# meuleman/epilogos

Hardware: AMD Instinct MI355X
Metric: Mbins scored/sec (S1, 18-state, 833 biosamples) (higher is better)
Workload: dtype u8

## Files before the change

epilogos_amd/csrc/epg_common.h:

```cpp
#pragma once
#include <hip/hip_runtime.h>
#include <stdarg.h>
#include <stdint.h>
#include <stdio.h>

#include <type_traits>

#include "epilogos_amd.h"

typedef unsigned int u32;
typedef unsigned long long u64;
typedef unsigned short u16;

namespace epg {

int fail(int code, const char* fmt, ...);
int num_cus();

#ifdef EPILOGOS_BUILD_EXPERIMENTS
#include <stdlib.h>
static inline const char* exp_env(const char* name) { return getenv(name); }
#else
static inline const char* exp_env(const char*) { return nullptr; }
#endif

enum Force { FORCE_NULL_SEQ = 0, FORCE_S3_SCORE_BINS, FORCE_S3_CONTRACTION, FORCE_S3_HIST_LDS, FORCE_K1_BLOCKS_PER_CU, FORCE_CUS, FORCE_COUNT };
extern int g_force[FORCE_COUNT];

#define EPG_HIP(expr)                                                                         \
    do {                                                                                      \
        hipError_t _e = (expr);                                                               \
        if (_e != hipSuccess)                                                                 \
            return epg::fail(EPG_ERR_HIP, "%s failed: %s", #expr, hipGetErrorString(_e));     \
    } while (0)

#define EPG_LAUNCH_CHECK(name)                                                                \
    do {                                                                                      \
        hipError_t _e = hipGetLastError();                                                    \
        if (_e != hipSuccess)                                                                 \
            return epg::fail(EPG_ERR_HIP, "launch of %s failed: %s", name, hipGetErrorString(_e)); \
    } while (0)

static inline int64_t align_up(int64_t x, int64_t a) { return (x + a - 1) / a * a; }

template <int DEFAULT, typename F>
static inline auto with_constant(int, F&& f) {
    return f(std::integral_constant<int, DEFAULT>{});
}
template <int DEFAULT, int V, int... VS, typename F>
static inline auto with_constant(int v, F&& f) {
    if (v == V) return f(std::integral_constant<int, V>{});
    return with_constant<DEFAULT, VS...>(v, f);
}

int64_t s1_ws_bytes(int64_t R, int N, int S);
int grid_for_tiles(long R);
long fast_rows(long R, int N, long ldx);
int64_t s2_table_bytes(int maxc, int S);
int64_t s3_ws_bytes(int64_t R, int N, int S);
int64_t s3_xt_bytes(int64_t R, int N);
int transpose_states(const char* X, int64_t R, int32_t N, int64_t ldx, int32_t S, char* XT, int64_t Rp, int shift, int bad, int* dirty,
                     hipStream_t st);
int64_t s3_gemm_ws_bytes(int64_t R, int N, int S);
int64_t s3_gemm_ws_min_bytes(int64_t R, int N, int S);
int hist_s3_gemm(const char* X, int64_t R, int32_t N, int64_t ldx, int32_t S, int32_t* counts, void* ws, int64_t ws_bytes, hipStream_t st);
bool s3_lanes_ok(int N, int S);
int64_t s3_lanes_ws_bytes(int64_t R, int N, int S);
int score_s3_lanes(const int8_t* X8, int64_t R, int32_t N, int64_t ldx, int32_t S, const float* q, double* out64, float* out32, void* ws,
                   int64_t ws_bytes, hipStream_t st);
int wide_hist_s2_from_binhist(const uint16_t* H, const uint16_t* H2, int64_t R, int32_t S, int64_t* counts, hipStream_t st);
int wide_score_s2_from_hist(const uint16_t* H, int64_t R, int32_t S, int64_t perms, const float* q, double* out64, float* out32, hipStream_t st);
int wide_hist_s3(const int8_t* X, int64_t R, int32_t N, int64_t ldx, int32_t S, int32_t* counts, hipStream_t st);
int wide_score_s3(const int8_t* X, int64_t R, int32_t N, int64_t ldx, int32_t S, const float* q, double* out64, float* out32, void* ws,
                  int64_t ws_bytes, hipStream_t st);

struct DynLds {
    unsigned long long done = 0;
};
static inline hipError_t ensure_dyn_lds(DynLds& a, const void* kernel, int bytes) {
    int dev = 0;
    hipError_t e = hipGetDevice(&dev);
    if (e != hipSuccess) return e;
    const unsigned long long bit = 1ull << (dev & 63);
    if (__atomic_load_n(&a.done, __ATOMIC_ACQUIRE) & bit) return hipSuccess;
    e = hipFuncSetAttribute(kernel, hipFuncAttributeMaxDynamicSharedMemorySize, bytes);
    if (e == hipSuccess) __atomic_fetch_or(&a.done, bit, __ATOMIC_RELEASE);
    return e;
}

static inline int tile_rows(int64_t row_bytes) {
    int tr = 64;
    while (tr > 8 && 4 * tr * row_bytes > 65536) tr >>= 1;
    return tr;
}

__device__ __forceinline__ u32 bfi(u32 m, u32 a, u32 b) { return (a & m) | (b & ~m); }

__device__ __forceinline__ uint4 ld16(const char* p) {
    uint4 v;
    __builtin_memcpy(&v, p, 16);
    return v;
}

__device__ __forceinline__ u32 quad_sum(u32 v) {
    v += (u32)__builtin_amdgcn_update_dpp(0, (int)v, 0xB1, 0xf, 0xf, false);
    v += (u32)__builtin_amdgcn_update_dpp(0, (int)v, 0x4E, 0xf, 0xf, false);
    return v;
}

__device__ __forceinline__ void store_staged(const char* lds, char* dst, int nbytes, int lane) {
    const int nchunks = nbytes >> 4;
    for (int c = lane; c < nchunks; c += 64)
        *reinterpret_cast<uint4*>(dst + 16 * c) = *reinterpret_cast<const uint4*>(lds + 16 * c);
    const int tail0 = nchunks << 4;
    for (int o = tail0 + 4 * lane; o + 4 <= nbytes; o += 256)
        *reinterpret_cast<u32*>(dst + o) = *reinterpret_cast<const u32*>(lds + o);
    if ((nbytes & 2) && lane == 0) *reinterpret_cast<u16*>(dst + nbytes - 2) = *reinterpret_cast<const u16*>(lds + nbytes - 2);
}

typedef u32 epg_u32x4 __attribute__((ext_vector_type(4)));
__device__ __forceinline__ void store_staged_nt(const char* lds, char* dst, int nbytes, int lane) {
    const int nchunks = nbytes >> 4;
    for (int c = lane; c < nchunks; c += 64)
        __builtin_nontemporal_store(*reinterpret_cast<const epg_u32x4*>(lds + 16 * c), reinterpret_cast<epg_u32x4*>(dst + 16 * c));
    const int tail0 = nchunks << 4;
    for (int o = tail0 + 4 * lane; o + 4 <= nbytes; o += 256)
        __builtin_nontemporal_store(*reinterpret_cast<const u32*>(lds + o), reinterpret_cast<u32*>(dst + o));
    if ((nbytes & 2) && lane == 0) *reinterpret_cast<u16*>(dst + nbytes - 2) = *reinterpret_cast<const u16*>(lds + nbytes - 2);
}

__device__ __forceinline__ double kl_term(double p, double q) {
    if (q == 0.0) return 0.0;
    const double r = p / q;
    if (!(r > 0.0)) return 0.0;
    return p * log2(r);
}

__device__ __forceinline__ float s3_table_entry(float qv, float obs) {
    if (qv == 0.0f) return 0.0f;
    const float r = __fdiv_rn(obs, qv);
    if (!(r > 0.0f)) return 0.0f;
#ifdef EPG_S3_TABLE_LOG2F
    return obs * log2f(r);
#else
    return __fmul_rn(obs, (float)log2((double)r));
#endif
}

}
```

epilogos_amd/csrc/epg_s1.hip:

```cpp
#include "epg_count.h"
#include "epg_paircount.h"

#include <stdlib.h>
#include <string.h>

namespace epg {

constexpr int K1P_LD = 17;

template <int SC, bool FULL, bool PAIRS, typename Loop>
__device__ __forceinline__ void bin_hist_body(int Sout_, u64* __restrict__ counts, int nmax, u64* __restrict__ counts2, Loop&& loop) {
    constexpr int S = SC;
    constexpr int ND = (S + 1) / 2;
    const int Sout = FULL ? S : Sout_;
    const int ROWB = 2 * Sout;
    __shared__ u64 s_cnt[S + 1];
    __shared__ __attribute__((aligned(16))) char s_stage[4][32 * 2 * S];
    constexpr int PG = (S + 2) / 3, PSP = 3 * PG, PROLES = PG * (PG + 1) / 2, PSLICE = PROLES <= 64 ? 64 / PROLES : 1;
    static_assert(!PAIRS || (FULL && PROLES <= 64), "the pair counts need a compile-time row width and at most 64 block roles");
    __shared__ u32 s_pair[PAIRS ? 4 * PSP * K1P_LD : 1];
    __shared__ u64 s_c2[PAIRS ? S * S : 1];
    const int lane = threadIdx.x & 63, wave = threadIdx.x >> 6;
    const int j = lane & 3, b = lane >> 2;
    if (threadIdx.x <= S) s_cnt[threadIdx.x] = 0;
    if (PAIRS) {
        for (int e = threadIdx.x; e < S * S; e += 256) s_c2[e] = 0;
        for (int e = threadIdx.x; e < 4 * PSP * K1P_LD; e += 256) s_pair[e] = 0;
    }
    __syncthreads();
    u16* H = nullptr;
    int pgi = -1, pgj = 0, pkq = 0;
    u64 pacc[PAIRS ? 9 : 1], prs[PAIRS ? 3 : 1];
    if (PAIRS) {
        const int role = lane < PROLES * PSLICE ? lane / PSLICE : -1;
        pkq = lane % PSLICE;
        if (role >= 0) pair_role(role, PG, pgi, pgj);
#pragma unroll
        for (int c = 0; c < 9; ++c) pacc[c] = 0;
#pragma unroll
        for (int c = 0; c < 3; ++c) prs[c] = 0;
    }
    auto pair_counts = [&](const char* stage, int rows) {
        u32* sp = s_pair + wave * PSP * K1P_LD;
        const u16* raw = reinterpret_cast<const u16*>(stage);
        __builtin_amdgcn_wave_barrier();
        for (int e = lane; e < S * 16; e += 64) {
            const int i = e >> 4, k = e & 15;
            const u32 lo = 2 * k < rows ? raw[(2 * k) * S + i] : 0u, hi = 2 * k + 1 < rows ? raw[(2 * k + 1) * S + i] : 0u;
            sp[i * K1P_LD + k] = lo | (hi << 16);
        }
        __builtin_amdgcn_wave_barrier();
        if (pgi >= 0) {
            u32 part[9], ps[3];
            pair_tile_dot(sp + 3 * pgi * K1P_LD, sp + 3 * pgj * K1P_LD, K1P_LD, pkq, 16, PSLICE, pgi == pgj, part, ps);
#pragma unroll
            for (int c = 0; c < 9; ++c) pacc[c] += part[c];
#pragma unroll
            for (int c = 0; c < 3; ++c) prs[c] += ps[c];
        }
        __builtin_amdgcn_wave_barrier();
    };

    StateTotals<S> totals;
    totals.init(nmax);

    auto enter = [&](u16* Hpart) { H = Hpart; };
    auto epilogue = [&](int half, long row, bool valid, u32 (&cnt)[S]) {
        u32 d[ND];
        pack_reduce<S>(cnt, d);
        if (counts) totals.add(d, valid, s_cnt, j);
        if (H) stage_hist_row<S, FULL && (S & 1) == 0>(&s_stage[wave][(half * 16 + b) * ROWB], d, j, Sout);
    };
    auto finish = [&](long st, long row0, int rows) {
        if (H) store_staged(s_stage[wave], reinterpret_cast<char*>(H) + row0 * ROWB, rows * ROWB, lane);
        if constexpr (PAIRS) pair_counts(s_stage[wave], rows);
    };
    loop(enter, epilogue, finish);

    if (counts) totals.commit(s_cnt, j, counts, Sout);
    if constexpr (PAIRS) {
        if (pgi >= 0) pair_fold(pacc, prs, pgi, pgj, S, s_c2);
        pair_commit(s_c2, S, counts2);
    }
}

template <int SC, int NG, bool FULL>
__global__ __launch_bounds__(256) void k_bin_hist(const char* __restrict__ X, long R, int N, long ldx, int Sout_,
                                                   u16* __restrict__ H, u64* __restrict__ counts) {
    bin_hist_body<SC, FULL, false>(Sout_, counts, N, nullptr, [&](auto&& enter, auto&& epilogue, auto&& finish) {
        enter(H);
        tile_loop<SC, NG>(X, R, N, ldx, epilogue, finish);
    });
}

template <int SC, int NG>
__global__ __launch_bounds__(256) void k_bin_hist_s2(const char* __restrict__ X, long R, int N, long ldx, u16* __restrict__ H,
                                                      u64* __restrict__ counts, u64* __restrict__ counts2) {
    bin_hist_body<SC, true, true>(SC, counts, N, counts2, [&](auto&& enter, auto&& epilogue, auto&& finish) {
        enter(H);
        tile_loop<SC, NG>(X, R, N, ldx, epilogue, finish);
    });
}

template <int SC, int NG, bool FULL>
__global__ __launch_bounds__(256) void k_bin_hist_parts(const KhParts pt, int Sout_, u64* __restrict__ counts, int nmax) {
    bin_hist_body<SC, FULL, false>(Sout_, counts, nmax, nullptr, [&](auto&& enter, auto&& epilogue, auto&& finish) {
        tile_loop_parts<SC, NG>(pt, [&](int part) { enter(pt.h[part]); }, epilogue, finish);
    });
}

__global__ __launch_bounds__(256) void k_bin_hist_safe(const char* __restrict__ X, long row_begin, long row_end, int N,
                                                        long ldx, int S, u16* __restrict__ H, u64* __restrict__ counts, int mask = 31) {
    __shared__ u32 s_h[4][128];
    const int lane = threadIdx.x & 63, wave = threadIdx.x >> 6;
    for (long row = row_begin + (long)blockIdx.x * 4 + wave; row < row_end; row += (long)gridDim.x * 4) {
        for (int s = lane; s < S; s += 64) s_h[wave][s] = 0;
        __builtin_amdgcn_wave_barrier();
        const char* rp = X + row * ldx;
        for (int n = lane; n < N; n += 64) {
            const int v = (unsigned char)rp[n] & mask;
            if (v < S) atomicAdd(&s_h[wave][v], 1u);
        }
        __builtin_amdgcn_wave_barrier();
        for (int s = lane; s < S; s += 64) {
            const u32 c = s_h[wave][s];
            if (H) H[row * S + s] = (u16)c;
            if (counts && c) atomicAdd(&counts[s], (u64)c);
        }
        __builtin_amdgcn_wave_barrier();
    }
}

__global__ void k_s1_table(const float* __restrict__ q, int N, int S, double* __restrict__ T64, float* __restrict__ T32) {
    const long e = (long)blockIdx.x * blockDim.x + threadIdx.x;
    if (e >= (long)(N + 1) * S) return;
    const int c = (int)(e / S), s = (int)(e % S);
    const double p = (double)c / (double)N;
    const double v = kl_term(p, (double)q[s]);
    T64[e] = v;
    T32[e] = (float)v;
}

template <int S, int NG, typename OT>
__global__ __launch_bounds__(256) void k_score_s1(const char* __restrict__ X, long R, int N, long ldx,
                                                   const OT* __restrict__ T, OT* __restrict__ out) {
    constexpr int ND = (S + 1) / 2;
    constexpr int ROWB = S * (int)sizeof(OT);
    __shared__ __attribute__((aligned(16))) char s_stage[4][32 * ROWB];
    const int lane = threadIdx.x & 63, wave = threadIdx.x >> 6;
    const int j = lane & 3, b = lane >> 2;
    auto epilogue = [&](int half, long row, bool valid, u32 (&cnt)[S]) {
        u32 d[ND];
        pack_reduce<S>(cnt, d);
        OT* srow = reinterpret_cast<OT*>(&s_stage[wave][(half * 16 + b) * ROWB]);
#pragma unroll
        for (int k = 0; k < (S + 3) / 4; ++k) {
            const u32 c = quad_state_count(d, k, j);
            const int s = 4 * k + j;
            if (s < S) srow[s] = (c && valid) ? T[(long)c * S + s] : (OT)0;
        }
    };
    auto finish = [&](long st, long row0, int rows) {
        store_staged_nt(s_stage[wave], reinterpret_cast<char*>(out) + row0 * ROWB, rows * ROWB, lane);
    };
    tile_loop<S, NG>(X, R, N, ldx, epilogue, finish);
}

template <typename OT, bool LDS_T>
__global__ __launch_bounds__(LDS_T ? 1024 : 256) void k_score_s1_from_hist(const u16* __restrict__ H, long total, int S,
                                                                             const OT* __restrict__ Tg, int nent, OT* __restrict__ out,
                                                                             u64* __restrict__ zero_counts, int rev) {
    extern __shared__ __attribute__((aligned(16))) char smem_t[];
    if (zero_counts && blockIdx.x == 0 && (int)threadIdx.x < S) zero_counts[threadIdx.x] = 0;
    const OT* T = Tg;
    if (LDS_T) {
        OT* Ts = reinterpret_cast<OT*>(smem_t);
        for (int e = threadIdx.x; e < nent; e += blockDim.x) Ts[e] = Tg[e];
        __syncthreads();
        T = Ts;
    }
    const u32 cmax = (u32)(nent / S - 1);
    const long nquads = total >> 2;
    const long stride = (long)gridDim.x * blockDim.x;
    long qd = (long)blockIdx.x * blockDim.x + threadIdx.x;
    const long qtop = nquads - 1, qsgn = rev ? -1 : 1, qoff = rev ? qtop : 0;
    for (; qd + 3 * stride < nquads; qd += 4 * stride) {
        uint2 h[4];
#pragma unroll
        for (int u = 0; u < 4; ++u) h[u] = *reinterpret_cast<const uint2*>(H + 4 * (qoff + qsgn * (qd + u * stride)));
#pragma unroll
        for (int u = 0; u < 4; ++u) {
            const long e0 = 4 * (qoff + qsgn * (qd + u * stride));
            int s = (int)(e0 % S);
            const u32 c[4] = {h[u].x & 0xffffu, h[u].x >> 16, h[u].y & 0xffffu, h[u].y >> 16};
            OT v[4];
#pragma unroll
            for (int k = 0; k < 4; ++k) {
                v[k] = c[k] - 1u < cmax ? T[(long)c[k] * S + s] : (OT)0;
                s = s + 1 == S ? 0 : s + 1;
            }
            if constexpr (sizeof(OT) == 4) {
                typedef float v4f_nt __attribute__((ext_vector_type(4)));
                const v4f_nt vv = {(float)v[0], (float)v[1], (float)v[2], (float)v[3]};
                __builtin_nontemporal_store(vv, reinterpret_cast<v4f_nt*>(out + e0));
            } else {
                typedef double v2d_nt __attribute__((ext_vector_type(2)));
                const v2d_nt lo = {(double)v[0], (double)v[1]}, hi = {(double)v[2], (double)v[3]};
                __builtin_nontemporal_store(lo, reinterpret_cast<v2d_nt*>(out + e0));
                __builtin_nontemporal_store(hi, reinterpret_cast<v2d_nt*>(out + e0 + 2));
            }
        }
    }
    for (; qd < nquads; qd += stride) {
        const long e0 = 4 * (qoff + qsgn * qd);
        int s = (int)(e0 % S);
        for (int k = 0; k < 4; ++k) {
            const u32 c = H[e0 + k];
            out[e0 + k] = c - 1u < cmax ? T[(long)c * S + s] : (OT)0;
            s = s + 1 == S ? 0 : s + 1;
        }
    }
    if (blockIdx.x == 0 && threadIdx.x < (total & 3)) {
        const long e = (nquads << 2) + threadIdx.x;
        const u32 c = H[e];
        out[e] = c - 1u < cmax ? T[(long)c * S + (int)(e % S)] : (OT)0;
    }
}

template <typename IT>
__global__ __launch_bounds__(256) void k_sum_int(const IT* __restrict__ C, long n, long long* __restrict__ total) {
    long long acc = 0;
    for (long i = (long)blockIdx.x * blockDim.x + threadIdx.x; i < n; i += (long)gridDim.x * blockDim.x) acc += (long long)C[i];
    for (int off = 32; off > 0; off >>= 1) acc += __shfl_down(acc, off);
    __shared__ long long s_part[4];
    if ((threadIdx.x & 63) == 0) s_part[threadIdx.x >> 6] = acc;
    __syncthreads();
    if (threadIdx.x == 0) {
        const long long t = s_part[0] + s_part[1] + s_part[2] + s_part[3];
        if (t) atomicAdd(reinterpret_cast<u64*>(total), (u64)t);
    }
}

template <typename IT>
__global__ __launch_bounds__(256) void k_normalise(const IT* __restrict__ C, long n, const long long* __restrict__ total,
                                                    float* __restrict__ q) {
    const double tot = (double)(*total);
    for (long i = (long)blockIdx.x * blockDim.x + threadIdx.x; i < n; i += (long)gridDim.x * blockDim.x)
        q[i] = (float)((double)C[i] / tot);
}

template <typename IT>
__global__ __launch_bounds__(256) void k_normalise_small(const IT* __restrict__ C, int n, float* __restrict__ q) {
    __shared__ long long s_part[4];
    long long acc = 0;
    for (int i = threadIdx.x; i < n; i += 256) acc += (long long)C[i];
    for (int off = 32; off > 0; off >>= 1) acc += __shfl_down(acc, off);
    if ((threadIdx.x & 63) == 0) s_part[threadIdx.x >> 6] = acc;
    __syncthreads();
    const double tot = (double)(s_part[0] + s_part[1] + s_part[2] + s_part[3]);
    for (int i = threadIdx.x; i < n; i += 256) q[i] = (float)((double)C[i] / tot);
}

static int blocks_per_cu() { return g_force[FORCE_K1_BLOCKS_PER_CU] > 0 ? g_force[FORCE_K1_BLOCKS_PER_CU] : 2; }
int grid_for_tiles(long R) {
    const long nsuper = (R + 31) >> 5;
    long blocks = (nsuper + 3) / 4;
    const long cap = (long)num_cus() * blocks_per_cu();
    if (blocks > cap) {
        const long iters = (nsuper + cap * 4 - 1) / (cap * 4);
        blocks = (nsuper + iters * 4 - 1) / (iters * 4);
    }
    if (blocks < 1) blocks = 1;
    return (int)blocks;
}

template <typename F>
static void with_count_core(int S, int ng, F&& f) {
    if (S == 15 || S == 18 || S == 25)
        with_constant<25, 15, 18>(S, [&](auto sc) {
            with_constant<0, 1, 2, 3, 4, 5, 6, 7, 8>(ng, [&](auto NG) { f(sc, NG, std::true_type{}); });
        });
    else
        with_constant<31, 15, 18, 25>(S < 15 ? 15 : S < 18 ? 18 : S < 25 ? 25 : 31,
                                      [&](auto sc) { f(sc, std::integral_constant<int, 0>{}, std::false_type{}); });
}

long fast_rows(long R, int N, long ldx) {
    const long chunks = (N + 15) / 16;
    const long over = 16 * chunks - ldx;
    if (over <= 0) return R;
    const long unsafe = (over + ldx - 1) / ldx;
    return R > unsafe ? R - unsafe : 0;
}

extern "C" int epg_bin_hist(const int8_t* X8, int64_t R, int32_t N, int64_t ldx, int32_t S, uint16_t* H, int64_t* counts, void* stream) {
    hipStream_t st = (hipStream_t)stream;
    if (R < 0 || N < 1 || ldx < N || S < 1) return fail(EPG_ERR_INVALID_ARG, "bin_hist: bad shape R=%lld N=%d ldx=%lld S=%d", (long long)R, N, (long long)ldx, S);
    if (S > 127) return fail(EPG_ERR_UNSUPPORTED, "bin_hist: S=%d > 127 (states are int8)", S);
    if (N > 65535) return fail(EPG_ERR_UNSUPPORTED, "bin_hist: N=%d > 65535 (uint16 per-bin counts)", N);
    if (R == 0) return EPG_OK;
    if (!X8) return fail(EPG_ERR_INVALID_ARG, "bin_hist: X is NULL");
    if (H && (reinterpret_cast<uintptr_t>(H) & 15)) return fail(EPG_ERR_INVALID_ARG, "bin_hist: H must be 16-byte aligned");
    const char* X = reinterpret_cast<const char*>(X8);
    u64* cnt = reinterpret_cast<u64*>(counts);
    if (S > 31) {
        hipLaunchKernelGGL(k_bin_hist_safe, dim3((unsigned)((R + 3) / 4 < num_cus() * 32L ? (R + 3) / 4 : num_cus() * 32L)), dim3(256), 0, st, X, 0L,
                           (long)R, N, ldx, S, H, cnt, 255);
        EPG_LAUNCH_CHECK("k_bin_hist_safe");
        return EPG_OK;
    }
    const long Rf = fast_rows(R, N, ldx);
    if (Rf > 0) {
        with_count_core(S, (N + 127) / 128, [&](auto SC, auto NG, auto MODEL) {
            hipLaunchKernelGGL((k_bin_hist<SC, NG, MODEL && (SC & 1) == 0>), dim3(grid_for_tiles(Rf)), dim3(256), 0, st, X, Rf, N, ldx, S, H, cnt);
        });
        EPG_LAUNCH_CHECK("k_bin_hist");
    }
    if (Rf < R) {
        hipLaunchKernelGGL(k_bin_hist_safe, dim3((unsigned)((R - Rf + 3) / 4 < 1024 ? (R - Rf + 3) / 4 : 1024)), dim3(256), 0, st, X, Rf, (long)R, N, ldx, S, H, cnt);
        EPG_LAUNCH_CHECK("k_bin_hist_safe");
    }
    return EPG_OK;
}

extern "C" int epg_bin_hist_s2(const int8_t* X8, int64_t R, int32_t N, int64_t ldx, int32_t S, uint16_t* H, int64_t* counts, int64_t* counts2,
                               void* stream) {
    hipStream_t st = (hipStream_t)stream;
    if (!H || !counts2) return fail(EPG_ERR_INVALID_ARG, "bin_hist_s2: H and counts2 are required");
    const bool fused = (S == 15 || S == 18 || S == 25) && R > 0 && N >= 1 && N <= 1024 && ldx >= N && X8 &&
                       !(reinterpret_cast<uintptr_t>(H) & 15) && fast_rows(R, N, ldx) == R;
    if (!fused) {
        int rc = epg_bin_hist(X8, R, N, ldx, S, H, counts, stream);
        if (rc) return rc;
        return epg_hist_s2_from_binhist(H, R, S, counts2, stream);
    }
    const char* X = reinterpret_cast<const char*>(X8);
    u64* c1 = reinterpret_cast<u64*>(counts);
    u64* c2 = reinterpret_cast<u64*>(counts2);
    with_constant<25, 18, 15>(S, [&](auto SC) {
        with_constant<8, 1, 2, 3, 4, 5, 6, 7>((N + 127) / 128, [&](auto NG) {
            hipLaunchKernelGGL((k_bin_hist_s2<decltype(SC)::value, NG>), dim3(grid_for_tiles(R)), dim3(256), 0, st, X, R, N, ldx, H, c1, c2);
        });
    });
    EPG_LAUNCH_CHECK("k_bin_hist_s2");
    return EPG_OK;
}

extern "C" int epg_bin_hist_parts(int32_t nparts, const int8_t* const* X, const int64_t* R, const int32_t* N, const int64_t* ldx, int32_t S,
                                  uint16_t* const* H, int64_t* counts, void* stream) {
    hipStream_t st = (hipStream_t)stream;
    if (nparts < 0 || (nparts && (!X || !R || !N || !ldx))) return fail(EPG_ERR_INVALID_ARG, "bin_hist_parts: NULL argument array");
    if (S < 1 || S > 127) return fail(EPG_ERR_UNSUPPORTED, "bin_hist_parts: S=%d outside 1..127", S);
    for (int p = 0; p < nparts; ++p) {
        if (R[p] < 0 || (R[p] && (N[p] < 1 || ldx[p] < N[p]))) return fail(EPG_ERR_INVALID_ARG, "bin_hist_parts: bad shape of part %d", p);
        if (R[p] && N[p] > 65535) return fail(EPG_ERR_UNSUPPORTED, "bin_hist_parts: N=%d > 65535 (uint16 per-bin counts)", N[p]);
        if (R[p] && !X[p]) return fail(EPG_ERR_INVALID_ARG, "bin_hist_parts: X of part %d is NULL", p);
        if (H && H[p] && (reinterpret_cast<uintptr_t>(H[p]) & 15)) return fail(EPG_ERR_INVALID_ARG, "bin_hist_parts: H of part %d must be 16-byte aligned", p);
    }
    if (S > 31) {
        for (int p = 0; p < nparts; ++p) {
            const int rc = epg_bin_hist(X[p], R[p], N[p], ldx[p], S, H ? H[p] : nullptr, counts, stream);
            if (rc) return rc;
        }
        return EPG_OK;
    }
    u64* cnt = reinterpret_cast<u64*>(counts);
    for (int p = 0; p < nparts; ++p) {
        const long Rf = R[p] ? fast_rows(R[p], N[p], ldx[p]) : 0;
        if (Rf == R[p]) continue;
        hipLaunchKernelGGL(k_bin_hist_safe, dim3((unsigned)((R[p] - Rf + 3) / 4 < 1024 ? (R[p] - Rf + 3) / 4 : 1024)), dim3(256), 0, st,
                           reinterpret_cast<const char*>(X[p]), Rf, (long)R[p], N[p], (long)ldx[p], S, H ? H[p] : nullptr, cnt);
        EPG_LAUNCH_CHECK("k_bin_hist_safe");
    }
    auto cls = [](int n) { const int ng = (n + 127) / 128; return ng <= 8 ? ng : 0; };
    for (int c = 0; c <= 8; ++c) {
        for (int p0 = 0; p0 < nparts;) {
            KhParts pt;
            int nmax = 1;
            p0 = pack_parts(pt, p0, nparts, 32, [&](int p) { return R[p] && cls(N[p]) == c ? fast_rows(R[p], N[p], ldx[p]) : 0L; },
                            [&](int k, int p) {
                                pt.x[k] = reinterpret_cast<const char*>(X[p]); pt.h[k] = H ? H[p] : nullptr;
                                pt.ldx[k] = ldx[p]; pt.n_cols[k] = N[p];
                                if (N[p] > nmax) nmax = N[p];
                            });
            if (pt.n == 0) break;
            with_count_core(S, c, [&](auto SC, auto NG, auto) {
                hipLaunchKernelGGL((k_bin_hist_parts<SC, NG, (NG > 0 && (SC & 1) == 0)>), dim3(grid_for_tiles(pt.t0[pt.n] * 32)), dim3(256), 0, st, pt, S,
                                   cnt, nmax);
            });
            EPG_LAUNCH_CHECK("k_bin_hist_parts");
        }
    }
    return EPG_OK;
}

static int64_t s1_table_bytes(int N, int S) { return align_up((int64_t)(N + 1) * S * 8, 256) + align_up((int64_t)(N + 1) * S * 4, 256); }

int64_t s1_ws_bytes(int64_t R, int N, int S) {
    return s1_table_bytes(N, S) + 256 + align_up(R * S * 2, 256);
}

static int build_s1_table(const float* q, int N, int S, void* ws, double** T64, float** T32, hipStream_t st) {
    *T64 = reinterpret_cast<double*>(ws);
    *T32 = reinterpret_cast<float*>(reinterpret_cast<char*>(ws) + align_up((int64_t)(N + 1) * S * 8, 256));
    const long n = (long)(N + 1) * S;
    hipLaunchKernelGGL(k_s1_table, dim3((int)((n + 255) / 256)), dim3(256), 0, st, q, N, S, *T64, *T32);
    EPG_LAUNCH_CHECK("k_s1_table");
    return EPG_OK;
}
static int check_score_from_hist_args(const uint16_t* H, const double* out64, const float* out32) {
    if ((reinterpret_cast<uintptr_t>(H) & 7) != 0) return fail(EPG_ERR_INVALID_ARG, "score_s1_from_binhist: H must be 8-byte aligned");
    if ((out32 && (reinterpret_cast<uintptr_t>(out32) & 15)) || (out64 && (reinterpret_cast<uintptr_t>(out64) & 15)))
        return fail(EPG_ERR_INVALID_ARG, "score_s1_from_binhist: outputs must be 16-byte aligned");
    return EPG_OK;
}

template <typename OT>
static int launch_score_s1_from_hist_t(const uint16_t* H, long total, int32_t S, const OT* T, int nent, OT* out, u64* zero_counts, hipStream_t st) {
    const size_t tbytes = (size_t)nent * sizeof(OT);
    const int rev = 1;
    if (tbytes <= 150 * 1024) {
        const int per_cu = tbytes <= 75 * 1024 ? 2 : 1;
        long nb = (total / 4 + 4095) / 4096;
        if (nb > (long)num_cus() * per_cu) nb = (long)num_cus() * per_cu;
        if (nb < 1) nb = 1;
        auto kern = k_score_s1_from_hist<OT, true>;
        static DynLds lds_attr;
        EPG_HIP(ensure_dyn_lds(lds_attr, reinterpret_cast<const void*>(kern), 150 * 1024));
        hipLaunchKernelGGL(kern, dim3((int)nb), dim3(1024), tbytes, st, H, total, S, T, nent, out, zero_counts, rev);
    } else {
        long nb = (total / 4 + 1023) / 1024;
        if (nb > num_cus() * 8L) nb = num_cus() * 8L;
        if (nb < 1) nb = 1;
        hipLaunchKernelGGL((k_score_s1_from_hist<OT, false>), dim3((int)nb), dim3(256), 0, st, H, total, S, T, nent, out, zero_counts, rev);
    }
    EPG_LAUNCH_CHECK("k_score_s1_from_hist");
    return EPG_OK;
}

static int launch_score_s1_from_hist(const uint16_t* H, int64_t R, int32_t N, int32_t S, const double* T64, const float* T32,
                                     double* out64, float* out32, hipStream_t st, u64* zero_counts = nullptr) {
    const long total = (long)R * S;
    const int nent = (N + 1) * S;
    int rc = EPG_OK;
    if (out32) rc = launch_score_s1_from_hist_t<float>(H, total, S, T32, nent, out32, zero_counts, st);
    if (!rc && out64) rc = launch_score_s1_from_hist_t<double>(H, total, S, T64, nent, out64, out32 ? nullptr : zero_counts, st);
    return rc;
}


extern "C" int epg_score_s1_from_binhist(const uint16_t* H, int64_t R, int32_t N, int32_t S, const float* q, double* out64, float* out32,
                                         void* ws, int64_t ws_bytes, void* stream) {
    hipStream_t st = (hipStream_t)stream;
    if (R < 0 || N < 1 || S < 1) return fail(EPG_ERR_INVALID_ARG, "score_s1: bad shape");
    if (R == 0) return EPG_OK;
    if (!H || !q || !ws) return fail(EPG_ERR_INVALID_ARG, "score_s1_from_binhist: NULL argument");
    if (ws_bytes < s1_table_bytes(N, S)) return fail(EPG_ERR_WORKSPACE, "score_s1: workspace %lld < %lld bytes", (long long)ws_bytes, (long long)s1_table_bytes(N, S));
    int rc = check_score_from_hist_args(H, out64, out32);
    if (rc) return rc;
    double* T64; float* T32;
    rc = build_s1_table(q, N, S, ws, &T64, &T32, st);
    if (rc) return rc;
    return launch_score_s1_from_hist(H, R, N, S, T64, T32, out64, out32, st);
}

extern "C" int epg_score_s1_from_binhist_table(const uint16_t* H, int64_t R, int32_t N, int32_t S, const double* T64, const float* T32,
                                               double* out64, float* out32, void* stream) {
    if (R < 0 || N < 1 || S < 1) return fail(EPG_ERR_INVALID_ARG, "score_s1: bad shape");
    if (R == 0) return EPG_OK;
    if (!H || (out64 && !T64) || (out32 && !T32)) return fail(EPG_ERR_INVALID_ARG, "score_s1_from_binhist_table: NULL argument");
    if ((T64 && (reinterpret_cast<uintptr_t>(T64) & 7)) || (T32 && (reinterpret_cast<uintptr_t>(T32) & 3)))
        return fail(EPG_ERR_INVALID_ARG, "score_s1_from_binhist_table: misaligned table");
    int rc = check_score_from_hist_args(H, out64, out32);
    if (rc) return rc;
    return launch_score_s1_from_hist(H, R, N, S, T64, T32, out64, out32, (hipStream_t)stream);
}

__global__ __launch_bounds__(256) void k_s1_combine(const u64* __restrict__ counts, int N, int S, float* __restrict__ q,
                                                     double* __restrict__ T64, float* __restrict__ T32) {
    __shared__ long long s_c[128];
    __shared__ double s_q[128];
    const int t = threadIdx.x;
    if (t < S) s_c[t] = (long long)counts[t];
    __syncthreads();
    if (t < S) {
        long long tot = 0;
        for (int s = 0; s < S; ++s) tot += s_c[s];
        const float qf = (float)((double)s_c[t] / (double)tot);
        if (blockIdx.x == 0) q[t] = qf;
        s_q[t] = (double)qf;
    }
    __syncthreads();
    const int e = blockIdx.x * 256 + t;
    if (e < (N + 1) * S) {
        const int c = e / S, s = e - c * S;
        const double v = kl_term((double)c / (double)N, s_q[s]);
        T64[e] = v;
        T32[e] = (float)v;
    }
}

extern "C" int epg_combine_score_s1(int64_t* counts, int32_t rezero, const uint16_t* H, int64_t R, int32_t N, int32_t S, float* q,
                                    double* out64, float* out32, void* ws, int64_t ws_bytes, void* stream) {
    hipStream_t st = (hipStream_t)stream;
    if (R < 0 || N < 1 || S < 1) return fail(EPG_ERR_INVALID_ARG, "combine_score_s1: bad shape R=%lld N=%d S=%d", (long long)R, N, S);
    if (S > 127) return fail(EPG_ERR_UNSUPPORTED, "combine_score_s1: S=%d > 127 (states are int8)", S);
    if (!counts || !q || !ws || (R > 0 && !H)) return fail(EPG_ERR_INVALID_ARG, "combine_score_s1: NULL argument");
    if (ws_bytes < s1_table_bytes(N, S)) return fail(EPG_ERR_WORKSPACE, "combine_score_s1: workspace %lld < %lld bytes", (long long)ws_bytes, (long long)s1_table_bytes(N, S));
    int rc = check_score_from_hist_args(H, out64, out32);
    if (rc) return rc;
    double* T64 = reinterpret_cast<double*>(ws);
    float* T32 = reinterpret_cast<float*>(reinterpret_cast<char*>(ws) + align_up((int64_t)(N + 1) * S * 8, 256));
    const long nent = (long)(N + 1) * S;
    hipLaunchKernelGGL(k_s1_combine, dim3((unsigned)((nent + 255) / 256)), dim3(256), 0, st, reinterpret_cast<const u64*>(counts), N, S, q, T64, T32);
    EPG_LAUNCH_CHECK("k_s1_combine");
    if (R == 0 || (!out32 && !out64)) {
        if (rezero) EPG_HIP(hipMemsetAsync(counts, 0, (size_t)S * 8, st));
        return EPG_OK;
    }
    return launch_score_s1_from_hist(H, R, N, S, T64, T32, out64, out32, st, rezero ? reinterpret_cast<u64*>(counts) : nullptr);
}

extern "C" int epg_hist_s1(const int8_t* X, int64_t R, int32_t N, int64_t ldx, int32_t S, int64_t* counts, void* stream) {
    if (!counts) return fail(EPG_ERR_INVALID_ARG, "hist_s1: counts is NULL");
    return epg_bin_hist(X, R, N, ldx, S, nullptr, counts, stream);
}

extern "C" int epg_score_s1(const int8_t* X8, int64_t R, int32_t N, int64_t ldx, int32_t S, const float* q, double* out64, float* out32,
                            void* ws, int64_t ws_bytes, void* stream) {
    hipStream_t st = (hipStream_t)stream;
    if (R < 0 || N < 1 || ldx < N || S < 1) return fail(EPG_ERR_INVALID_ARG, "score_s1: bad shape");
    if (S > 127) return fail(EPG_ERR_UNSUPPORTED, "score_s1: S=%d > 127 (states are int8)", S);
    if (R == 0) return EPG_OK;
    if (!X8 || !q || !ws) return fail(EPG_ERR_INVALID_ARG, "score_s1: NULL argument");
    if ((out32 && (reinterpret_cast<uintptr_t>(out32) & 15)) || (out64 && (reinterpret_cast<uintptr_t>(out64) & 15)))
        return fail(EPG_ERR_INVALID_ARG, "score_s1: outputs must be 16-byte aligned");
    const long Rf = fast_rows(R, N, ldx);
    const bool fused = S == 18 && Rf == R;
    if (!fused) {
        if (ws_bytes < s1_ws_bytes(R, N, S)) return fail(EPG_ERR_WORKSPACE, "score_s1: workspace %lld < %lld bytes", (long long)ws_bytes, (long long)s1_ws_bytes(R, N, S));
        u16* H = reinterpret_cast<u16*>(reinterpret_cast<char*>(ws) + s1_table_bytes(N, S));
        int rc = epg_bin_hist(X8, R, N, ldx, S, H, nullptr, stream);
        if (rc) return rc;
        return epg_score_s1_from_binhist(H, R, N, S, q, out64, out32, ws, s1_table_bytes(N, S), stream);
    }
    if (ws_bytes < s1_table_bytes(N, S)) return fail(EPG_ERR_WORKSPACE, "score_s1: workspace %lld < %lld bytes", (long long)ws_bytes, (long long)s1_table_bytes(N, S));
    double* T64; float* T32;
    int rc = build_s1_table(q, N, S, ws, &T64, &T32, st);
    if (rc) return rc;
    const char* X = reinterpret_cast<const char*>(X8);
    with_constant<0, 1, 2, 3, 4, 5, 6, 7, 8>((N + 127) / 128, [&](auto NG) {
        if (out32) hipLaunchKernelGGL((k_score_s1<18, NG, float>), dim3(grid_for_tiles(R)), dim3(256), 0, st, X, R, N, ldx, T32, out32);
        if (out64) hipLaunchKernelGGL((k_score_s1<18, NG, double>), dim3(grid_for_tiles(R)), dim3(256), 0, st, X, R, N, ldx, T64, out64);
    });
    EPG_LAUNCH_CHECK("k_score_s1");
    return EPG_OK;
}

template <typename IT>
static int normalise_impl(const IT* C, int64_t n, float* q, void* ws, int64_t ws_bytes, hipStream_t st) {
    if (n < 1 || !C || !q || !ws) return fail(EPG_ERR_INVALID_ARG, "normalise: bad argument");
    if (ws_bytes < 8) return fail(EPG_ERR_WORKSPACE, "normalise: workspace needs 8 bytes");
    if (n <= 4096) {
        hipLaunchKernelGGL((k_normalise_small<IT>), dim3(1), dim3(256), 0, st, C, (int)n, q);
        EPG_LAUNCH_CHECK("k_normalise_small");
        return EPG_OK;
    }
    long long* total = reinterpret_cast<long long*>(ws);
    EPG_HIP(hipMemsetAsync(total, 0, 8, st));
    long blocks = (n + 255) / 256;
    if (blocks > num_cus() * 8L) blocks = num_cus() * 8L;
    hipLaunchKernelGGL((k_sum_int<IT>), dim3((int)blocks), dim3(256), 0, st, C, (long)n, total);
    hipLaunchKernelGGL((k_normalise<IT>), dim3((int)blocks), dim3(256), 0, st, C, (long)n, total, q);
    EPG_LAUNCH_CHECK("k_normalise");
    return EPG_OK;
}

extern "C" int epg_normalise_i64(const int64_t* C, int64_t n, float* q, void* ws, int64_t ws_bytes, void* stream) {
    return normalise_impl<long long>(reinterpret_cast<const long long*>(C), n, q, ws, ws_bytes, (hipStream_t)stream);
}
extern "C" int epg_normalise_i32(const int32_t* C, int64_t n, float* q, void* ws, int64_t ws_bytes, void* stream) {
    return normalise_impl<int>(C, n, q, ws, ws_bytes, (hipStream_t)stream);
}

}
```

Measured before the change: 5763.

## Add specialized f32 S1 score kernel with padded LDS table and vectorized staging

Adds a float-only S1 scoring kernel. It pads the LDS lookup table with zero rows at count 0 and count N+1, so the branchy validity check becomes a clamp, and it precomputes per-thread state offsets so the per-element modulo goes away. Loads are issued 8 quads at a time per thread to keep more memory requests in flight. The table staging in both kernels now uses 16-byte vectorized global loads. The change adds a new code path that is selected by default for float outputs, and it assumes S<=1024 and a fixed state phase per thread stride.

```diff
diff --git a/epilogos_amd/csrc/epg_common.h b/epilogos_amd/csrc/epg_common.h
--- a/epilogos_amd/csrc/epg_common.h
+++ b/epilogos_amd/csrc/epg_common.h
@@ -24,7 +24,7 @@
 static inline const char* exp_env(const char*) { return nullptr; }
 #endif
 
-enum Force { FORCE_NULL_SEQ = 0, FORCE_S3_SCORE_BINS, FORCE_S3_CONTRACTION, FORCE_S3_HIST_LDS, FORCE_K1_BLOCKS_PER_CU, FORCE_CUS, FORCE_COUNT };
+enum Force { FORCE_NULL_SEQ = 0, FORCE_S3_SCORE_BINS, FORCE_S3_CONTRACTION, FORCE_S3_HIST_LDS, FORCE_K1_BLOCKS_PER_CU, FORCE_CUS, FORCE_S1_SCORE_GENERAL, FORCE_COUNT };
 extern int g_force[FORCE_COUNT];
 
 #define EPG_HIP(expr)                                                                         \
diff --git a/epilogos_amd/csrc/epg_s1.hip b/epilogos_amd/csrc/epg_s1.hip
--- a/epilogos_amd/csrc/epg_s1.hip
+++ b/epilogos_amd/csrc/epg_s1.hip
@@ -166,6 +166,37 @@
     tile_loop<S, NG>(X, R, N, ldx, epilogue, finish);
 }
 
+
+constexpr int STAGE_THREADS = 1024, STAGE_MAXV = 10;
+template <typename OT>
+__device__ __forceinline__ void stage_table(const OT* __restrict__ Tg, OT* __restrict__ Ts, int first, int last) {
+    constexpr int PER = 16 / (int)sizeof(OT);
+    typedef OT vec_t __attribute__((ext_vector_type(PER)));
+    const int t = threadIdx.x;
+    int head = (int)((16 - (reinterpret_cast<uintptr_t>(Tg + first) & 15)) & 15) / (int)sizeof(OT);
+    if (head > last - first) head = last - first;
+    const int v0 = first + head, nvec = (last - v0) / PER, tail0 = v0 + nvec * PER;
+    vec_t v[STAGE_MAXV];
+    OT eh = 0, et = 0;
+#pragma unroll
+    for (int j = 0; j < STAGE_MAXV; ++j) {
+        const int i = t + j * STAGE_THREADS;
+        if (i < nvec) v[j] = *reinterpret_cast<const vec_t*>(Tg + v0 + i * PER);
+    }
+    if (t < head) eh = Tg[first + t];
+    if (t < last - tail0) et = Tg[tail0 + t];
+#pragma unroll
+    for (int j = 0; j < STAGE_MAXV; ++j) {
+        const int i = t + j * STAGE_THREADS;
+        if (i < nvec) {
+#pragma unroll
+            for (int k = 0; k < PER; ++k) Ts[v0 + i * PER + k] = v[j][k];
+        }
+    }
+    if (t < head) Ts[first + t] = eh;
+    if (t < last - tail0) Ts[tail0 + t] = et;
+}
+
 template <typename OT, bool LDS_T>
 __global__ __launch_bounds__(LDS_T ? 1024 : 256) void k_score_s1_from_hist(const u16* __restrict__ H, long total, int S,
                                                                              const OT* __restrict__ Tg, int nent, OT* __restrict__ out,
@@ -175,7 +206,7 @@
     const OT* T = Tg;
     if (LDS_T) {
         OT* Ts = reinterpret_cast<OT*>(smem_t);
-        for (int e = threadIdx.x; e < nent; e += blockDim.x) Ts[e] = Tg[e];
+        stage_table<OT>(Tg, Ts, 0, nent);
         __syncthreads();
         T = Ts;
     }
@@ -224,6 +255,72 @@
         const long e = (nquads << 2) + threadIdx.x;
         const u32 c = H[e];
         out[e] = c - 1u < cmax ? T[(long)c * S + (int)(e % S)] : (OT)0;
+    }
+}
+
+constexpr int S1F_FLY = 8;
+__global__ __launch_bounds__(1024) void k_score_s1_from_hist_f32(const u16* __restrict__ H, long total, int S, int N,
+                                                                  const float* __restrict__ Tg, float* __restrict__ out,
+                                                                  u64* __restrict__ zero_counts, int rev) {
+    extern __shared__ __attribute__((aligned(16))) char smem_t[];
+    typedef float v4f_nt __attribute__((ext_vector_type(4)));
+    if (zero_counts && blockIdx.x == 0 && (int)threadIdx.x < S) zero_counts[threadIdx.x] = 0;
+    float* Ts = reinterpret_cast<float*>(smem_t);
+    stage_table<float>(Tg, Ts, S, (N + 1) * S);
+    for (int s = threadIdx.x; s < S; s += blockDim.x) {
+        Ts[s] = 0.0f;
+        Ts[(N + 1) * S + s] = 0.0f;
+    }
+    __syncthreads();
+
+    const u32 cap = (u32)N + 1u, rowb = (u32)S * 4u;
+    const long nquads = total >> 2;
+    const u32 g4 = (u32)(S & -S) < 4u ? (u32)(S & -S) : 4u;
+    const u32 P = (u32)S / g4;
+    const u32 nall = gridDim.x * blockDim.x;
+    const u32 p64 = (P & (0u - P)) < 64u ? (P & (0u - P)) : 64u;
+    const u32 PW = P / p64 * 64u <= nall ? P / p64 * 64u : P;
+    const long nthr = (long)(nall - nall % PW);
+    const long g = (long)blockIdx.x * blockDim.x + threadIdx.x;
+    const long qsgn = rev ? -1 : 1;
+    long qfirst = g, left = g < nquads ? (nquads - 1 - g) / nthr + 1 : 0;
+    if (rev) {
+        const long top = (nquads + 63) & ~63L;
+        qfirst = top - 1 - g;
+        if (qfirst >= nquads) qfirst -= nthr;
+        left = qfirst >= 0 ? qfirst / nthr + 1 : 0;
+    }
+    if (g < nthr && left > 0) {
+        const u32 s0 = (u32)((4 * qfirst) % S);
+        u32 off[4];
+#pragma unroll
+        for (int k = 0; k < 4; ++k) off[k] = ((s0 + (u32)k) % (u32)S) * 4u;
+        auto score_quad = [&](const uint2 h, float* o) {
+            const u32 c[4] = {h.x & 0xffffu, h.x >> 16, h.y & 0xffffu, h.y >> 16};
+            v4f_nt v;
+#pragma unroll
+            for (int k = 0; k < 4; ++k) {
+                const u32 cc = c[k] < cap ? c[k] : cap;
+                v[k] = *reinterpret_cast<const float*>(smem_t + (__umul24(cc, rowb) + off[k]));
+            }
+            __builtin_nontemporal_store(v, reinterpret_cast<v4f_nt*>(o));
+        };
+        const long step = qsgn * nthr * 4;
+        const u16* hp = H + 4 * qfirst;
+        float* op = out + 4 * qfirst;
+        for (; left >= S1F_FLY; left -= S1F_FLY, hp += S1F_FLY * step, op += S1F_FLY * step) {
+            uint2 h[S1F_FLY];
+#pragma unroll
+            for (int u = 0; u < S1F_FLY; ++u) h[u] = *reinterpret_cast<const uint2*>(hp + u * step);
+#pragma unroll
+            for (int u = 0; u < S1F_FLY; ++u) score_quad(h[u], op + u * step);
+        }
+        for (; left > 0; --left, hp += step, op += step) score_quad(*reinterpret_cast<const uint2*>(hp), op);
+    }
+    if (blockIdx.x == 0 && threadIdx.x < (total & 3)) {
+        const long e = (nquads << 2) + threadIdx.x;
+        const u32 c = H[e];
+        out[e] = Ts[(c < cap ? c : cap) * (u32)S + (u32)(e % S)];
     }
 }
 
@@ -419,6 +516,20 @@
 static int launch_score_s1_from_hist_t(const uint16_t* H, long total, int32_t S, const OT* T, int nent, OT* out, u64* zero_counts, hipStream_t st) {
     const size_t tbytes = (size_t)nent * sizeof(OT);
     const int rev = 1;
+    if constexpr (std::is_same<OT, float>::value) {
+        const size_t fbytes = tbytes + 2 * (size_t)S * sizeof(float);
+        if (fbytes <= 150 * 1024 && S <= 1024 && !g_force[FORCE_S1_SCORE_GENERAL]) {
+            const int per_cu = fbytes <= 75 * 1024 ? 2 : 1;
+            long nb = (total / 4 + 4095) / 4096;
+            if (nb > (long)num_cus() * per_cu) nb = (long)num_cus() * per_cu;
+            if (nb < 1) nb = 1;
+            static DynLds lds_attr;
+            EPG_HIP(ensure_dyn_lds(lds_attr, reinterpret_cast<const void*>(k_score_s1_from_hist_f32), 150 * 1024));
+            hipLaunchKernelGGL(k_score_s1_from_hist_f32, dim3((int)nb), dim3(1024), fbytes, st, H, total, S, nent / S - 1, T, out, zero_counts, rev);
+            EPG_LAUNCH_CHECK("k_score_s1_from_hist_f32");
+            return EPG_OK;
+        }
+    }
     if (tbytes <= 150 * 1024) {
         const int per_cu = tbytes <= 75 * 1024 ? 2 : 1;
         long nb = (total / 4 + 4095) / 4096;
```

New measurement: 5850 (median of 6 runs). 1.5% higher.
